# lijingzhu1/SKGHOI

Hardware: AMD Instinct MI355X
Metric: images/sec through interaction head (20x20 pairs) (higher is better)
Workload: dtype f32; 1 GPU; HICO-DET-shaped synthetic cached detections: 20 humans x 20 objects per image (G=800 grid rows, P=780 pairs, K=117 verbs), eval forward of InteractionHead from cached AdaMixer-R50 box features [40,256,7,7]/image; precision=fp32, batch_per_gpu=256, parallelism=dp1 (independent image shards, no data-path collective)

## Files before the change

include/skghoi.h:

```cpp
#ifndef SKGHOI_H
#define SKGHOI_H
#include <stdint.h>
#ifdef __cplusplus
extern "C" {
#endif

#define SKG_ABI_VERSION 19
#define SKG_E_ARG   (-1)
#define SKG_E_ALIGN (-2)
#define SKG_E_LIMIT (-3)
#define SKG_E_UNSUPPORTED (-4)
#define SKG_E_COMM  (-5)

#define SKG_MAX_DET_PER_IMAGE 1024
#define SKG_MAX_NODES         160
#define SKG_SPATIAL_LD        48
#define SKG_TRANSH_DIM        50
#define SKG_TRANSH_ENT        80

int         skg_abi_version(void);
const char* skg_build_info(void);

typedef struct {
    int32_t image;
// ... 117 lines not shown
int skg_gemm_dot_partials(const skg_gemm_desc* desc_host);

#define SKG_GEMM_GROUP_MAX 4
int skg_gemm_group_f32(const skg_gemm_desc* descs_host, int n, void* stream);
int skg_gemm_group_tile(const skg_gemm_desc* descs_host, int n);
int skg_gemm_b16_f32(const skg_gemm_desc* desc_host, const uint16_t* w16, void* stream);
int skg_gemm_group_b16_f32(const skg_gemm_desc* descs_host, const uint16_t* const* w16_host, int n, void* stream);
int skg_gemm_b16_a16_f32(const skg_gemm_desc* desc_host, const uint16_t* a16, const uint16_t* w16, void* stream);
void skg_gemm_b16_a16_launches(int64_t* out_host, int reset);
typedef struct {
    const uint16_t* w16;
    const uint16_t* a16;
    uint16_t*       c16; int64_t ldc16;
} skg_gemm_b16_io;
int  skg_gemm_b16_x(const skg_gemm_desc* desc_host, const skg_gemm_b16_io* io, void* stream);
int  skg_gemm_group_b16_x(const skg_gemm_desc* descs_host, const skg_gemm_b16_io* ios, int n, void* stream);
void skg_gemm_b16_x_counts(int64_t* out3, int reset);
#define SKG_GEMM_PATH_EXACT  0
#define SKG_GEMM_PATH_FP16X2 1
#define SKG_GEMM_PATH_BF16   2
#define SKG_GEMM_PATH_ROUTED 3
#define SKG_GEMM_PATHS       4
void skg_gemm_path_counts(int64_t* out_host, int reset);
typedef struct { int32_t small_mode, small_tiles, route_tiles, khalves_blocks; } skg_tuning;

int skg_concat_entity_f32(const float* enc, int64_t ld_enc, const int32_t* enc_row, const float* ent,
                          const int32_t* ent_img, const int32_t* ent_row, int rows, float* out, int64_t out_ld,
                          void* stream);
int skg_concat_entity_x(const float* enc, int64_t ld_enc, const int32_t* enc_row, const float* ent,
                        const int32_t* ent_img, const int32_t* ent_row, int rows, void* out, int64_t out_ld,
                        int out_dtype, void* stream);

typedef struct {
    const uint16_t* A; int64_t lda;
    const uint16_t* W; int64_t ldw;
    const float* bias;
    void* C; int64_t ldc;
    int32_t M, N, K;
    int32_t relu, out_bf16, split_k;
    float* split_ws;
} skg_gemm_bf16_desc;
int skg_gemm_bf16(const skg_gemm_bf16_desc* desc_host, void* stream);
int skg_transpose_bf16(const void* in, int64_t ld_in, int rows, int cols, void* out, int64_t ld_out, void* stream);

int skg_transpose_f32(const float* in, int64_t ld_in, int rows, int cols, float* out, int64_t ld_out, void* stream);

int skg_rows_mul_relu_f32(const float* P, const int32_t* p_idx, int64_t ldp, const float* Q, const int32_t* q_idx,
// ... 275 lines not shown
```

skghoi_amd/_capi.py:

```python
import ctypes as C
import os

_HERE = os.path.dirname(os.path.abspath(__file__))
LIB_PATH = os.environ.get("SKG_LIB") or os.path.join(_HERE, "csrc", "libskghoi_hip.so")

EPI_BIAS, EPI_BIAS_RELU, EPI_MUL_RELU, EPI_RELU_DOT, EPI_BIAS_RES_RELU = range(5)
DTYPE_F32, DTYPE_F16, DTYPE_BF16 = range(3)
DTYPE_BYTES = 3
CACHE_MAX_ARRAYS, CACHE_MAX_BATCH = 16, 256
MAX_DET_PER_IMAGE = 1024
MAX_NODES = 160
SPATIAL_LD = 48
TRANSH_DIM = 50
TRANSH_ENT = 80
ABI_VERSION = 19
GEMM_GROUP_MAX = 4
CHECKSUM_PARTIALS = 1024
LOSS_CHUNKS = 64

_vp = C.c_void_p
_i32 = C.c_int32
_i64 = C.c_int64
_f32 = C.c_float


class GemmDesc(C.Structure):
    _fields_ = [("A", _vp), ("lda", _i64), ("W", _vp), ("ldw", _i64), ("bias", _vp), ("C", _vp), ("ldc", _i64),
                ("M", _i32), ("N", _i32), ("K", _i32), ("epilogue", _i32), ("a_rows", _vp), ("out_rows", _vp),
                ("P", _vp), ("p_idx", _vp), ("ldp", _i64), ("Q", _vp), ("q_idx", _vp), ("ldq", _i64),
                ("mbias", _vp), ("C_raw", _vp), ("ldc_raw", _i64), ("dot_w", _vp), ("dot_partial", _vp),
                ("res", _vp), ("ldres", _i64), ("split_k", _i32), ("w_scale", _f32), ("split_ws", _vp), ("w_split", _vp),
                ("a_exp", _vp)]


class GemmB16Io(C.Structure):
    _fields_ = [("w16", _vp), ("a16", _vp), ("c16", _vp), ("ldc16", _i64)]


class GemmXDesc(C.Structure):
# ... 94 lines not shown
                                  _vp, C.c_int, C.c_int, C.c_int, _vp, C.c_int, _vp]),
    "skg_roi_align_nhwc_x": (C.c_int, [_vp, C.c_int, _vp, _vp, _vp, C.c_int, C.c_int, C.c_int, C.c_int, _f32, C.c_int,
                                       _vp, _vp, C.c_int, C.c_int, C.c_int, _vp, C.c_int, _vp]),
    "skg_roi_align_bwd_nhwc_f32": (C.c_int, [_vp, _vp, _vp, _vp, C.c_int, C.c_int, C.c_int, C.c_int, _f32, C.c_int, _vp,
                                             _vp, C.c_int, C.c_int, C.c_int, _vp, _vp]),
    "skg_roi_align_layout_counts": (None, [C.POINTER(_i64), C.c_int]),
    "skg_roi_align_bwd_det_x": (C.c_int, [_vp, C.c_int, _vp, _vp, _vp, C.c_int, C.c_int, C.c_int, C.c_int, _f32, C.c_int,
                                          _vp, _vp, C.c_int, C.c_int, C.c_int, C.c_int, _vp, _vp]),
    "skg_roi_align_bwd_det_nhwc_x": (C.c_int, [_vp, C.c_int, _vp, _vp, _vp, C.c_int, C.c_int, C.c_int, C.c_int, _f32,
                                               C.c_int, _vp, _vp, C.c_int, C.c_int, C.c_int, C.c_int, _vp, _vp]),
    "skg_roi_align_det_counts": (None, [C.POINTER(_i64), C.c_int]),
    "skg_global_avgpool_f32": (C.c_int, [_vp, C.c_int, C.c_int, C.c_int, _vp, _vp]),
    "skg_gemm_f32": (C.c_int, [C.POINTER(GemmDesc), _vp]),
    "skg_transh_draw_f32": (C.c_int, [_vp, _i64, C.c_int, C.c_int, C.c_int, C.c_int, _vp, _vp, _vp]),
    "skg_transh_draw_train_f32": (C.c_int, [_vp, _i64, C.c_int, C.c_int, C.c_int, _vp, _vp, _vp, _vp, _vp, _vp]),
    "skg_gemm_dot_partials": (C.c_int, [C.POINTER(GemmDesc)]),
    "skg_split_weights_bytes": (C.c_int64, [C.c_int, C.c_int]),
    "skg_split_weights_f16x2": (C.c_int, [_vp, C.c_int, C.c_int, _i64, _f32, _vp, _vp]),
    "skg_gemm_group_f32": (C.c_int, [C.POINTER(GemmDesc), C.c_int, _vp]),
    "skg_gemm_group_tile": (C.c_int, [C.POINTER(GemmDesc), C.c_int]),
    "skg_gemm_b16_f32": (C.c_int, [C.POINTER(GemmDesc), _vp, _vp]),
    "skg_gemm_group_b16_f32": (C.c_int, [C.POINTER(GemmDesc), C.POINTER(_vp), C.c_int, _vp]),
    "skg_gemm_path_counts": (None, [C.POINTER(_i64), C.c_int]),
    "skg_gemm_b16_a16_f32": (C.c_int, [C.POINTER(GemmDesc), _vp, _vp, _vp]),
    "skg_gemm_b16_a16_launches": (None, [C.POINTER(_i64), C.c_int]),
    "skg_gemm_b16_x": (C.c_int, [C.POINTER(GemmDesc), C.POINTER(GemmB16Io), _vp]),
    "skg_gemm_group_b16_x": (C.c_int, [C.POINTER(GemmDesc), C.POINTER(GemmB16Io), C.c_int, _vp]),
    "skg_gemm_b16_x_counts": (None, [C.POINTER(_i64), C.c_int]),
    "skg_row_exponents_f32": (C.c_int, [_vp, C.c_int64, _vp, C.c_int, C.c_int, _vp, _vp]),
    "skg_adamw_f32": (C.c_int, [_vp, C.c_int] + [C.c_double] * 7 + [_vp, C.c_int, _vp]),
    "skg_grad_sumsq_f32": (C.c_int, [_vp, C.c_int, _vp, _vp]),
    "skg_adamw_guarded_f32": (C.c_int, [_vp, C.c_int] + [C.c_double] * 7 + [_i64, C.c_double, C.c_int, _vp, C.c_int, _vp,
                                                                          C.c_int, _vp, _vp]),
    "skg_sizeof_step_status": (C.c_int, []),
    "skg_ctx_set_tuning": (C.c_int, [_vp, C.POINTER(Tuning)]),
    "skg_ctx_get_tuning": (C.c_int, [_vp, C.POINTER(Tuning)]),
    "skg_ctx_make_current": (_vp, [_vp]),
    "skg_gemmx_ws_floats": (C.c_int64, [C.POINTER(GemmXDesc)]),
    "skg_gemmx_f32": (C.c_int, [C.POINTER(GemmXDesc), C.c_int, _vp]),
    "skg_gemmx_bf16": (C.c_int, [C.POINTER(GemmXDesc), C.c_int, _vp]),
    "skg_gemmx_path_counts": (None, [C.POINTER(_i64), C.c_int]),
    "skg_gemm_bf16": (C.c_int, [C.POINTER(GemmBf16Desc), _vp]),
    "skg_transpose_bf16": (C.c_int, [_vp, _i64, C.c_int, C.c_int, _vp, _i64, _vp]),
    "skg_transpose_f32": (C.c_int, [_vp, _i64, C.c_int, C.c_int, _vp, _i64, _vp]),
    "skg_concat_entity_f32": (C.c_int, [_vp, _i64, _vp, _vp, _vp, _vp, C.c_int, _vp, _i64, _vp]),
    "skg_concat_entity_x": (C.c_int, [_vp, _i64, _vp, _vp, _vp, _vp, C.c_int, _vp, _i64, C.c_int, _vp]),
# ... 152 lines not shown
```

skghoi_amd/csrc/skg_common.h:

```cpp
#pragma once
#include <hip/hip_runtime.h>
#include <stdint.h>
#include "skghoi.h"

#define SKG_WAVE 64

typedef float f32x16 __attribute__((ext_vector_type(16)));
typedef float f32x4 __attribute__((ext_vector_type(4)));

static inline int skg_launch_status() {
    hipError_t e = hipGetLastError();
    return e == hipSuccess ? 0 : (int)e;
}

static inline bool skg_aligned16(const void* p) { return (((uintptr_t)p) & 15u) == 0; }
__device__ __forceinline__ bool skg_aligned16_dev(const void* p) { return (((uintptr_t)p) & 15u) == 0; }

__device__ __forceinline__ float skg_wave_sum(float v) {
#pragma unroll
    for (int off = 32; off > 0; off >>= 1) v += __shfl_xor(v, off, 64);
    return v;
}
__device__ __forceinline__ float skg_wave_max(float v) {
#pragma unroll
    for (int off = 32; off > 0; off >>= 1) v = fmaxf(v, __shfl_xor(v, off, 64));
    return v;
}

__device__ __forceinline__ float skg_block_sum256(float v, float* red) {
    v = skg_wave_sum(v);
    const int w = threadIdx.x >> 6;
    __syncthreads();
    if ((threadIdx.x & 63) == 0) red[w] = v;
    __syncthreads();
    return (red[0] + red[1]) + (red[2] + red[3]);
}

extern thread_local const skg_tuning* skg_tls_tuning;
static inline int skg_tune_small_mode() { const skg_tuning* t = skg_tls_tuning; return t && t->small_mode > 0 ? t->small_mode : 3; }
static inline int skg_tune_small_tiles() { const skg_tuning* t = skg_tls_tuning; return t && t->small_tiles > 0 ? t->small_tiles : 384; }
static inline int skg_tune_route_tiles() { const skg_tuning* t = skg_tls_tuning; return t && t->route_tiles > 0 ? t->route_tiles : 200; }
static inline int skg_tune_khalves_blocks() { const skg_tuning* t = skg_tls_tuning; return t && t->khalves_blocks > 0 ? t->khalves_blocks : 320; }

struct skg_twin_map { const float* base[2]; uint16_t* base16[2]; int64_t n[2]; };
extern thread_local skg_twin_map skg_tls_twin;
static inline uint16_t* skg_twin(const float* p) {
    const skg_twin_map& m = skg_tls_twin;
    for (int i = 0; i < 2; ++i)
        if (m.base16[i] && p >= m.base[i] && p < m.base[i] + m.n[i]) return m.base16[i] + (p - m.base[i]);
    return nullptr;
}
typedef __bf16 skg_bf2 __attribute__((ext_vector_type(2)));
typedef float skg_f2 __attribute__((ext_vector_type(2)));
__device__ __forceinline__ uint32_t skg_pack_bf16(float a, float b) {
    const skg_f2 v = {a, b};
    return __builtin_bit_cast(uint32_t, __builtin_convertvector(v, skg_bf2));
}
__device__ __forceinline__ void skg_store_twin4(uint16_t* p, const float4 v) {
    *reinterpret_cast<uint2*>(p) = make_uint2(skg_pack_bf16(v.x, v.y), skg_pack_bf16(v.z, v.w));
}

struct skg_gemmx_fused {
    int kind;
    const float* P; const int32_t* p_idx; int64_t ldp;
    const float* Q; const int32_t* q_idx; int64_t ldq;
    const float* mbias;
    float* C_raw; int64_t ldc_raw;
    const int32_t* out_rows;
    const float* res; int64_t ldres;
};
int skg_gemmx_can_fuse(const skg_gemmx_desc* d, const skg_gemmx_fused* f);
int skg_gemmx_f32_fused(const skg_gemmx_desc* descs_host, const skg_gemmx_fused* fused_host, int n, void* stream);

#define SKG_MULTI_MAX 4
struct skg_rows_mul_args {
    const float* P; const int32_t* p_idx; int64_t ldp; const float* Q; const int32_t* q_idx; int64_t ldq; const float* mbias;
    const float* F; const int32_t* f_idx; int64_t ldf; int rows, cols; float* out; int64_t ldo;
    uint16_t* out16;
};
int skg_rows_mul_relu_multi(const skg_rows_mul_args* calls, int n, void* stream);
struct skg_mul_bwd_args {
    float* g; int64_t ldg; const float* F; const int32_t* f_idx; int64_t ldf; const float* P; const int32_t* p_idx; int64_t ldp;
    const float* Q; const int32_t* q_idx; int64_t ldq; const float* mbias; int rows; float* dF; int64_t lddf; int accumulate;
    uint16_t* dF16;
};
int skg_mul_bwd_multi(const skg_mul_bwd_args* calls, int n, void* stream);
struct skg_segment_sum_args {
    const float* src; int64_t ld; int mode; float* outH; float* outN; int accumulate;
    uint16_t* outH16; uint16_t* outN16;
};
int skg_segment_sum_multi(const skg_segment_sum_args* calls, int n, const skg_image_meta* meta, const int32_t* hum_img,
                          const int32_t* node_img, int sum_h, int sum_n, void* stream);
struct skg_add_layernorm_args {
    const float* a; int64_t lda; const float* b; int64_t ldb; const float* gamma; const float* beta; int rows;
// ... 17 lines not shown
```

skghoi_amd/csrc/skg_gemm.hip:

```cpp
#include "skg_common.h"
#include <string.h>
#include <atomic>
#include <type_traits>

__device__ __forceinline__ float skg_exp2i(int e) { return __uint_as_float((uint32_t)(127 + e) << 23); }

typedef _Float16 f16x8 __attribute__((ext_vector_type(8)));
typedef _Float16 h16x2 __attribute__((ext_vector_type(2)));
typedef uint32_t u32x4 __attribute__((ext_vector_type(4)));
typedef short s16x8 __attribute__((ext_vector_type(8)));
typedef __bf16 bf16x2_t __attribute__((ext_vector_type(2)));
typedef float f32x2_t __attribute__((ext_vector_type(2)));

__device__ __forceinline__ uint32_t skg_pack_bf16x2(float a, float b) {
    const f32x2_t v = {a, b};
    return __builtin_bit_cast(uint32_t, __builtin_convertvector(v, bf16x2_t));
}
__device__ __forceinline__ void skg_store_bf16x4(uint16_t* p, float a, float b, float c, float e) {
    *reinterpret_cast<uint2*>(p) = make_uint2(skg_pack_bf16x2(a, b), skg_pack_bf16x2(c, e));
}
__device__ __forceinline__ void skg_store_bf16(uint16_t* p, float a) { *p = (uint16_t)(skg_pack_bf16x2(a, 0.f) & 0xffffu); }

#define BM 128
#define BN 128
// ... 1248 lines not shown
    if (d.split_k > 1 && (!d.split_ws || (d.epilogue != SKG_EPI_BIAS && d.epilogue != SKG_EPI_BIAS_RELU &&
                                          d.epilogue != SKG_EPI_BIAS_RES_RELU) || d.split_k > 64))
        return SKG_E_ARG;
    if (d.M < 0 || d.N <= 0 || d.K <= 0 || !d.A || !d.W) return SKG_E_ARG;
    if ((d.K & 3) || (d.lda & 3) || (d.ldw & 3)) return SKG_E_ALIGN;
    if (!skg_aligned16(d.A) || !skg_aligned16(d.W)) return SKG_E_ALIGN;
    if (d.lda < d.K && !d.a_rows && d.M > 1) return SKG_E_ARG;
    switch (d.epilogue) {
        case SKG_EPI_BIAS: case SKG_EPI_BIAS_RELU:
            if (!d.C) return SKG_E_ARG; break;
        case SKG_EPI_MUL_RELU:
            if (!d.C || (!d.P && !d.Q)) return SKG_E_ARG; break;
        case SKG_EPI_RELU_DOT:
            if (!d.dot_w || !d.dot_partial) return SKG_E_ARG; break;
        case SKG_EPI_BIAS_RES_RELU:
            if (!d.C || !d.res) return SKG_E_ARG; break;
        default: return SKG_E_ARG;
    }
    return 0;
}

#define g_route_tiles skg_tune_route_tiles()

static bool skg_route_desc(const skg_gemm_desc& d, skg_gemmx_desc& x, skg_gemmx_fused& f) {
    if (d.w_split || d.a_rows || d.a_exp || d.epilogue == SKG_EPI_RELU_DOT) return false;
    memset(&x, 0, sizeof(x)); memset(&f, 0, sizeof(f));
    x.A = d.A; x.a_sm = d.lda; x.a_sk = 1;
    x.B = d.W; x.b_sn = d.ldw; x.b_sk = 1;
    x.C = d.C; x.ldc = d.ldc; x.M = d.M; x.N = d.N; x.K = d.K;
    x.bias = d.bias; x.relu = d.epilogue == SKG_EPI_BIAS_RELU ? 1 : 0;
    x.split_k = d.split_k > 1 ? d.split_k : 0; x.split_ws = d.split_ws;
    f.out_rows = d.out_rows;
    if (d.epilogue == SKG_EPI_MUL_RELU) {
        f.kind = SKG_EPI_MUL_RELU;
        f.P = d.P; f.p_idx = d.p_idx; f.ldp = d.ldp; f.Q = d.Q; f.q_idx = d.q_idx; f.ldq = d.ldq; f.mbias = d.mbias;
        f.C_raw = d.C_raw; f.ldc_raw = d.ldc_raw;
    } else if (d.epilogue == SKG_EPI_BIAS_RES_RELU) {
        f.kind = SKG_EPI_BIAS_RES_RELU; f.res = d.res; f.ldres = d.ldres;
    }
    return skg_gemmx_can_fuse(&x, &f) != 0;
}

static bool skg_gemm_group_small(const skg_gemm_desc* descs, int n) {
    int64_t tiles128 = 0;
    for (int i = 0; i < n; ++i) {
        const skg_gemm_desc& d = descs[i];
        if (d.M == 0) continue;
        const bool glds = SKG_USE_GLDS && BK == 16 && (d.K % BK) == 0 && !d.a_rows &&
                          (int64_t)BM * d.lda * 4 < 0xffffffffLL && (int64_t)BN * d.ldw * 4 < 0xffffffffLL;
        if (!glds || (d.w_split && d.w_scale > 0.f)) return false;
        tiles128 += (int64_t)((d.M + 127) / 128) * ((d.N + 127) / 128);
    }
    return tiles128 < g_small_tiles;
}

static std::atomic<long long> g_gemm_path[SKG_GEMM_PATHS];
static inline void skg_gemm_count(int path) { g_gemm_path[path].fetch_add(1, std::memory_order_relaxed); }

extern "C" void skg_gemm_path_counts(int64_t* out_host, int reset) {
    for (int i = 0; i < SKG_GEMM_PATHS; ++i) {
        if (out_host) out_host[i] = g_gemm_path[i].load(std::memory_order_relaxed);
        if (reset) g_gemm_path[i].store(0, std::memory_order_relaxed);
    }
}

extern "C" int skg_gemm_group_tile(const skg_gemm_desc* descs_host, int n) {
    if (!descs_host || n < 1 || n > SKG_GEMM_GROUP_MAX) return SKG_E_ARG;
    return skg_gemm_group_small(descs_host, n) ? 1 : 2;
}

extern "C" int skg_gemm_group_f32(const skg_gemm_desc* descs_host, int n, void* stream) {
    if (!descs_host || n < 1 || n > SKG_GEMM_GROUP_MAX) return SKG_E_ARG;
    skg_gemm_group_args g, r;
    g.n = r.n = 0;
    int64_t blocks = 0, rblocks = 0;
    bool split = true;
    for (int i = 0; i < n; ++i) {
        const int rc = skg_gemm_validate(descs_host[i]);
        if (rc) return rc;
    }
    const bool small = skg_gemm_group_small(descs_host, n);
    if (n <= SKG_GEMMX_GROUP_MAX) {
        skg_gemmx_desc xs[SKG_GEMMX_GROUP_MAX];
        skg_gemmx_fused fs[SKG_GEMMX_GROUP_MAX];
        int64_t tiles128 = 0;
        bool ok = true;
        for (int i = 0; i < n && ok; ++i) {
            const skg_gemm_desc& d = descs_host[i];
            ok = skg_route_desc(d, xs[i], fs[i]);
            tiles128 += (int64_t)((d.M + 127) / 128) * ((d.N + 127) / 128) * (d.split_k > 1 ? d.split_k : 1);
        }
        if (ok && tiles128 >= g_route_tiles && tiles128 < 4 * g_small_tiles) {
            skg_gemm_count(SKG_GEMM_PATH_ROUTED);
            return skg_gemmx_f32_fused(xs, fs, n, stream);
        }
    }
    for (int i = 0; i < n; ++i) {
        const skg_gemm_desc& d = descs_host[i];
        if (d.split_k > 1 && !small) return SKG_E_ARG;
        if (d.M == 0) continue;
        split = split && d.w_split && (d.K % 16) == 0 && d.w_scale > 0.f;
        const int64_t nb = skg_gemm_blocks(d.M, d.N, d.K, small ? 1 : 2) * (d.split_k > 1 ? d.split_k : 1);
        if (blocks + nb > 0x7fffffffLL) return SKG_E_LIMIT;
        g.d[g.n] = d;
        g.start[g.n] = (int)blocks;
        blocks += nb;
        ++g.n;
        if (d.split_k > 1) {
            r.d[r.n] = d;
            r.start[r.n] = (int)rblocks;
            rblocks += ((int64_t)d.M * d.N + 255) / 256;
            ++r.n;
        }
    }
    if (g.n == 0) return 0;
// ... 5 lines not shown
    if (direct) hipLaunchKernelGGL(skg_gemm_group_direct_kernel, dim3((unsigned)blocks), dim3(256), 0, (hipStream_t)stream, g);
    else if (halves) hipLaunchKernelGGL(skg_gemm_group_khalves_kernel, dim3((unsigned)blocks), dim3(512), 0, (hipStream_t)stream, g);
    else if (small && g_small_mode >= 3) hipLaunchKernelGGL(skg_gemm_group_latency_kernel, dim3((unsigned)blocks), dim3(256), 0, (hipStream_t)stream, g);
    else if (small) hipLaunchKernelGGL(skg_gemm_group_small_kernel, dim3((unsigned)blocks), dim3(256), 0, (hipStream_t)stream, g);
    else if (split) hipLaunchKernelGGL(skg_gemm_group_split_kernel, dim3((unsigned)blocks), dim3(256), 0, (hipStream_t)stream, g);
    else hipLaunchKernelGGL(skg_gemm_group_kernel, dim3((unsigned)blocks), dim3(256), 0, (hipStream_t)stream, g);
    if (r.n) {
        for (int i = r.n; i <= SKG_GEMM_GROUP_MAX; ++i) r.start[i] = (int)rblocks;
        hipLaunchKernelGGL(skg_splitk_reduce_group_kernel, dim3((unsigned)rblocks), dim3(256), 0, (hipStream_t)stream, r);
    }
    return skg_launch_status();
}

extern "C" int skg_gemm_f32(const skg_gemm_desc* dh, void* stream) {
    if (!dh) return SKG_E_ARG;
    const skg_gemm_desc d = *dh;
    const int rc = skg_gemm_validate(d);
    if (rc) return rc;
    if (d.M == 0) return 0;
    const bool glds = SKG_USE_GLDS && BK == 16 && (d.K % BK) == 0 && !d.a_rows &&
                      (int64_t)BM * d.lda * 4 < 0xffffffffLL && (int64_t)BN * d.ldw * 4 < 0xffffffffLL;
    const bool split = d.w_split && (d.K % 16) == 0 && d.w_scale > 0.f;
    const int T = split ? 2 : skg_gemm_tile_scale(&d);
    if (!split && T == 1 && d.M > 64) {
        const int64_t tiles128 = (int64_t)((d.M + 127) / 128) * ((d.N + 127) / 128) * (d.split_k > 1 ? d.split_k : 1);
        skg_gemmx_desc x; skg_gemmx_fused f;
        if (tiles128 >= g_route_tiles && skg_route_desc(d, x, f)) {
            skg_gemm_count(SKG_GEMM_PATH_ROUTED);
            return skg_gemmx_f32_fused(&x, &f, 1, stream);
        }
    }
    const int64_t nblk = skg_gemm_blocks(d.M, d.N, d.K, T) * (d.split_k > 1 ? d.split_k : 1);
    if (nblk > 0x7fffffffLL) return SKG_E_LIMIT;
    dim3 grid((unsigned)nblk), block(256);
    hipStream_t s = (hipStream_t)stream;
    skg_gemm_count(split ? SKG_GEMM_PATH_FP16X2 : SKG_GEMM_PATH_EXACT);
#define SKG_LAUNCH(E)                                                                              \
    if (split) hipLaunchKernelGGL((skg_gemm_kernel<E, 2, 2>), grid, block, 0, s, d);               \
    else if (glds && T == 1 && g_small_mode == 4 && (d.K % 64) == 0) hipLaunchKernelGGL((skg_gemm_kernel<E, 4, 1>), grid, block, 0, s, d); \
    else if (glds && T == 1 && (g_small_mode == 5 || (g_small_mode == 6 && nblk <= g_khalves_blocks))) hipLaunchKernelGGL((skg_gemm_kernel<E, 5, 1>), grid, dim3(512), 0, s, d); \
    else if (glds && T == 1 && g_small_mode >= 3) hipLaunchKernelGGL((skg_gemm_kernel<E, 3, 1>), grid, block, 0, s, d); \
    else if (glds && T == 1) hipLaunchKernelGGL((skg_gemm_kernel<E, 1, 1>), grid, block, 0, s, d); \
    else if (glds) hipLaunchKernelGGL((skg_gemm_kernel<E, 1, 2>), grid, block, 0, s, d);           \
    else hipLaunchKernelGGL((skg_gemm_kernel<E, 0, 2>), grid, block, 0, s, d);
    switch (d.epilogue) {
        case SKG_EPI_BIAS:          SKG_LAUNCH(SKG_EPI_BIAS) break;
        case SKG_EPI_BIAS_RELU:     SKG_LAUNCH(SKG_EPI_BIAS_RELU) break;
        case SKG_EPI_MUL_RELU:      SKG_LAUNCH(SKG_EPI_MUL_RELU) break;
        case SKG_EPI_RELU_DOT:      SKG_LAUNCH(SKG_EPI_RELU_DOT) break;
        case SKG_EPI_BIAS_RES_RELU: SKG_LAUNCH(SKG_EPI_BIAS_RES_RELU) break;
// ... 306 lines not shown
```

skghoi_amd/csrc/skg_gemm_x.hip:

```cpp
#include "skg_common.h"
#include <stdlib.h>
#include <string.h>
#include <type_traits>
#include <atomic>

#define XBM 128
#define XBN 128
#define XBK 16
#define XLD 130
#define XTILE (XBK * XLD)
#ifndef SKG_XXCD
#define SKG_XXCD 1
#endif

struct skg_gemmx_group {
    skg_gemmx_desc d[SKG_GEMMX_GROUP_MAX];
    int start[SKG_GEMMX_GROUP_MAX + 1];
    skg_gemmx_fused f[SKG_GEMMX_GROUP_MAX];
    int vec[SKG_GEMMX_GROUP_MAX];
    int n;
};

__device__ __forceinline__ int64_t xoff(int idx, int shift, int64_t bstride, int64_t estride) {
    if (shift <= 0) return (int64_t)idx * estride;
// ... 169 lines not shown
}

template <bool WT = false>
__device__ __forceinline__ void xep_rows(const skg_gemmx_desc& d, const skg_gemmx_fused& f, const float* stage, int lane,
                                         int row0, int col0, float* ws) {
    const int c4 = 4 * (lane & 15), rr = lane >> 4, col = col0 + c4;
    if (col >= d.N) return;
    const bool hb = !ws && d.bias;
    float4 bv = xzero4(), mb = xzero4();
    if (hb) bv = xld4(d.bias + col);
    if (f.kind == SKG_EPI_MUL_RELU && f.mbias) mb = xld4(f.mbias + col);
    const int64_t coff = xoff(col, d.c_nshift, d.c_nstride, 1);
#pragma unroll
    for (int i = 0; i < 8; ++i) {
        const int row = row0 + 4 * i + rr;
        if (row >= d.M) continue;
        const float4 v = *reinterpret_cast<const float4*>(stage + (4 * i + rr) * XEP_LD + c4);
        if (WT) { xst_sc1(xrsrc(ws), ((uint32_t)row * (uint32_t)d.N + (uint32_t)col) * 4u, v); continue; }
        if (ws) { *reinterpret_cast<float4*>(ws + (int64_t)row * d.N + col) = v; continue; }
        xep_apply(d, f, v, row, col, coff, hb, bv, mb);
    }
}

template <bool OWN, int R>
__device__ __forceinline__ void xep_reduce(const skg_gemmx_desc& d, const skg_gemmx_fused& f, const float* stage, int lane,
                                           int row0, int col0, const XRed& red) {
    static_assert(R == 4 || R == 8, "rows per lane and pass");
    const int c4 = 4 * (lane & 15), rr = lane >> 4, col = col0 + c4;
    if (col >= d.N) return;
    const bool hb = d.bias != nullptr;
    float4 bv = xzero4(), mb = xzero4();
    if (hb) bv = xld4(d.bias + col);
    if (f.kind == SKG_EPI_MUL_RELU && f.mbias) mb = xld4(f.mbias + col);
    const int64_t coff = xoff(col, d.c_nshift, d.c_nstride, 1);
#pragma unroll 1
    for (int h = 0; h < 8 / R; ++h) {
        uint32_t ro[R];
        float4 sum[R];
#pragma unroll
        for (int i = 0; i < R; ++i) {
            ro[i] = ((uint32_t)min(row0 + 4 * (R * h + i) + rr, d.M - 1) * (uint32_t)d.N + (uint32_t)col) * 4u;
            sum[i] = xzero4();
        }
        auto add_slices = [&](int s0, int s1) {
            int s = s0;
            for (; s + 1 < s1; s += 2) {
// ... 247 lines not shown
    const bool split = S > 1;
    const int64_t MN = (int64_t)d.M * d.N;
    float* ws = split ? d.split_ws + (int64_t)slice * MN : nullptr;
    const bool inl = split && d.split_ctr != nullptr;
    if (c.do_rowsum && tid < XBM && m0 + tid < d.M) {
        if (split) xstore_rowsum_part(d.split_ws + (int64_t)S * MN + (int64_t)slice * d.M + m0 + tid, rsum, inl);
        else d.a_rowsum[m0 + tid] = d.accumulate ? d.a_rowsum[m0 + tid] + rsum : rsum;
    }
    if (vecbits & 8) {
        float* stage = smem + wave * XEP_WAVE;
#pragma unroll
        for (int ps = 0; ps < 2; ++ps) {
#pragma unroll
            for (int g2 = 0; g2 < 2; ++g2)
#pragma unroll
                for (int t = 0; t < 4; ++t)
#pragma unroll
                    for (int mb = 0; mb < 2; ++mb) {
                        const int e = 4 * (2 * ps + g2) + t;
                        *reinterpret_cast<float2*>(stage + (2 * (8 * g2 + 4 * lk + t) + mb) * XEP_LD + 2 * li) =
                            make_float2(acc[mb][0][e], acc[mb][1][e]);
                    }
            if (inl) xep_rows<true>(d, g.f[gi], stage, lane, m0 + wm * 64 + 32 * ps, n0 + wn * 64, ws);
            else xep_rows(d, g.f[gi], stage, lane, m0 + wm * 64 + 32 * ps, n0 + wn * 64, ws);
        }
        if (!inl || !xsplit_last(d.split_ctr + tm * nbn + tn, S, reinterpret_cast<uint32_t*>(smem + XEP_FLOATS))) return;
        if (c.do_rowsum && tid < XBM && m0 + tid < d.M) xreduce_rowsum_sc1(d, MN, m0 + tid);
        const XRed red = {d.split_ws, MN, S, -1};
#pragma unroll 1
        for (int ps = 0; ps < 2; ++ps)
            xep_reduce<false, 4>(d, g.f[gi], stage, lane, m0 + wm * 64 + 32 * ps, n0 + wn * 64, red);
        return;
    }
    const bool vecC = (vecbits >> 2) & 1;
    const int col = n0 + wn * 64 + 2 * li;
#pragma unroll
    for (int gq = 0; gq < 4; ++gq)
#pragma unroll
        for (int t = 0; t < 4; ++t)
#pragma unroll
            for (int mb = 0; mb < 2; ++mb) {
                const int row = m0 + wm * 64 + 2 * (8 * gq + 4 * lk + t) + mb;
                if (row >= d.M || col >= d.N) continue;
                float v0 = acc[mb][0][4 * gq + t], v1 = acc[mb][1][4 * gq + t];
                if (split) {
                    float* p = ws + (int64_t)row * d.N + col;
// ... 868 lines not shown
    if (quads) {
        const int64_t i = 4 * w;
        float4 v = xzero4();
        for (int s = 0; s < d.split_k; ++s) {
            const float4 q = xld4(d.split_ws + (int64_t)s * MN + i);
            v.x += q.x; v.y += q.y; v.z += q.z; v.w += q.w;
        }
        const int row = (int)(i / d.N), col = (int)(i % d.N);
        if (d.bias) { const float4 bv = xld4(d.bias + col); v.x += bv.x; v.y += bv.y; v.z += bv.z; v.w += bv.w; }
        if (d.relu) { v.x = fmaxf(v.x, 0.f); v.y = fmaxf(v.y, 0.f); v.z = fmaxf(v.z, 0.f); v.w = fmaxf(v.w, 0.f); }
        float* p = d.C + xoff(col, d.c_nshift, d.c_nstride, 1) + (int64_t)row * d.ldc;
        if (d.accumulate) { const float4 o = xld4(p); v.x += o.x; v.y += o.y; v.z += o.z; v.w += o.w; }
        if (d.mask) {
            const float4 m = xld4(d.mask + (int64_t)row * d.ldmask + col);
            v.x = m.x > 0.f ? v.x : 0.f; v.y = m.y > 0.f ? v.y : 0.f; v.z = m.z > 0.f ? v.z : 0.f; v.w = m.w > 0.f ? v.w : 0.f;
        }
        *reinterpret_cast<float4*>(p) = v;
        if (d.C16) *reinterpret_cast<uint2*>(d.C16 + (p - d.C)) = make_uint2(ypack(v.x, v.y), ypack(v.z, v.w));
        return;
    }
    xreduce_elem(d, MN, (int)(w / d.N), (int)(w % d.N));
}

static int skg_gemmx_validate(const skg_gemmx_desc& d) {
    if (d.M < 0 || d.N < 0 || d.K < 0) return SKG_E_ARG;
    if (d.M == 0 || d.N == 0) return 0;
    if (!d.C || d.ldc < 1) return SKG_E_ARG;
    if (d.K > 0 && (!d.A || !d.B)) return SKG_E_ARG;
    if (d.a_sm != 1 && d.a_sk != 1) return SKG_E_ARG;
    if (d.b_sn != 1 && d.b_sk != 1) return SKG_E_ARG;
    if (d.b_kshift < 0 || d.b_kshift > 30 || d.b_nshift < 0 || d.b_nshift > 30 || d.c_nshift < 0 || d.c_nshift > 30)
        return SKG_E_ARG;
    if ((d.b_kshift == 1) || (d.b_nshift == 1)) return SKG_E_ARG;
    if (d.mask && d.ldmask < d.N) return SKG_E_ARG;
    if (d.split_k > 1 && (!d.split_ws || d.split_k > 256)) return SKG_E_ARG;
    if ((((uintptr_t)d.C16) & 1u) || (((uintptr_t)d.A16) & 1u) || (((uintptr_t)d.B16) & 1u)) return SKG_E_ALIGN;
    if (((uintptr_t)d.split_ctr) & 3u) return SKG_E_ALIGN;
    if (d.a16_ld < 0 || d.b16_ld < 0 || (d.b16_ld && (d.b_kshift || d.b_nshift))) return SKG_E_ARG;
    if (d.a16_ld && d.a16_ld < (d.a_sk == 1 ? d.K : d.M)) return SKG_E_ARG;
    if (d.b16_ld && d.b16_ld < (d.b_sk == 1 ? d.K : d.N)) return SKG_E_ARG;
    return 0;
}

static bool xmul4(int64_t v) { return (v & 3) == 0; }
static bool xmul8(int64_t v) { return (v & 7) == 0; }

static int64_t xspan(int64_t idx, int shift, int64_t bstride, int64_t estride) {
    if (idx <= 0) return 0;
    if (shift <= 0) return idx * estride;
    return (idx >> shift) * bstride + (idx & ((1LL << shift) - 1)) * estride;
}
static bool xfits32(int64_t elems) { return elems >= 0 && elems < (1LL << 29); }

extern "C" int64_t skg_gemmx_ws_floats(const skg_gemmx_desc* d) {
    if (!d) return SKG_E_ARG;
    return d->split_k > 1 ? (int64_t)d->split_k * ((int64_t)d->M * d->N + d->M) : 0;
}

static bool xfused_ptrs_ok(const skg_gemmx_fused& f) {
    return skg_aligned16(f.P) && skg_aligned16(f.Q) && skg_aligned16(f.mbias) && skg_aligned16(f.C_raw) &&
           skg_aligned16(f.res) && xmul4(f.ldp) && xmul4(f.ldq) && xmul4(f.ldc_raw) && xmul4(f.ldres);
}

static std::atomic<long long> g_path_launches[3];
extern "C" void skg_gemmx_path_counts(int64_t* out3_host, int reset) {
    for (int i = 0; i < 3; ++i) {
        if (out3_host) out3_host[i] = g_path_launches[i].load(std::memory_order_relaxed);
        if (reset) g_path_launches[i].store(0, std::memory_order_relaxed);
    }
}

static bool g_t16_enabled = getenv("SKG_GEMMX_T16") == nullptr || atoi(getenv("SKG_GEMMX_T16")) != 0;

static int skg_gemmx_launch(const skg_gemmx_desc* descs_host, int n, void* stream, bool bf16,
                            const skg_gemmx_fused* fused_host = nullptr) {
    if (!descs_host || n < 1 || n > SKG_GEMMX_GROUP_MAX) return SKG_E_ARG;
    skg_gemmx_group g, r;
    memset(g.f, 0, sizeof(g.f)); memset(r.f, 0, sizeof(r.f));
    g.n = r.n = 0;
    int64_t blocks = 0, rblocks = 0;
    for (int i = 0; i < n; ++i) {
        const skg_gemmx_desc& d = descs_host[i];
        const int rc = skg_gemmx_validate(d);
        if (rc) return rc;
        if (d.M == 0 || d.N == 0) continue;
        const int S = d.split_k > 1 ? d.split_k : 1;
        const int64_t nb = (int64_t)((d.M + XBM - 1) / XBM) * ((d.N + XBN - 1) / XBN) * S;
        if (blocks + nb > 0x7fffffffLL) return SKG_E_LIMIT;
        int vec = 0;
        if (skg_aligned16(d.A) && (d.a_sk == 1 ? xmul4(d.a_sm) : xmul4(d.a_sk)) &&
            xfits32((int64_t)(d.M - 1) * d.a_sm + (int64_t)(d.K - 1) * d.a_sk + 4))
            vec |= 1;
        if (skg_aligned16(d.B) && (d.b_sk == 1 ? xmul4(d.b_sn) : xmul4(d.b_sk)) &&
            (d.b_kshift == 0 || (xmul4(d.b_kstride) && d.b_kshift >= 5)) && (d.b_nshift == 0 || xmul4(d.b_nstride)) &&
            xfits32(xspan(d.N - 1, d.b_nshift, d.b_nstride, d.b_sn) + xspan(d.K - 1, d.b_kshift, d.b_kstride, d.b_sk) + 4))
            vec |= 2;
        if ((((uintptr_t)d.C) & 7u) == 0 && (d.ldc & 1) == 0 && (d.c_nshift == 0 || (d.c_nstride & 1) == 0)) vec |= 4;
        if ((d.N & 3) == 0 && skg_aligned16(d.C) && xmul4(d.ldc) &&
            (d.c_nshift == 0 || (d.c_nshift >= 2 && xmul4(d.c_nstride))) && skg_aligned16(d.bias) &&
            skg_aligned16(d.mask) && (!d.mask || xmul4(d.ldmask)) && (S == 1 || skg_aligned16(d.split_ws)) &&
            (((uintptr_t)d.C16) & 7u) == 0)
            vec |= 8;
        const int64_t lda16 = d.a16_ld ? d.a16_ld : (d.a_sk == 1 ? d.a_sm : d.a_sk);
        const int64_t ldb16 = d.b16_ld ? d.b16_ld : (d.b_sk == 1 ? d.b_sn : d.b_sk);
        if (bf16 && d.A16 && ((vec & 1) || d.a16_ld) && skg_aligned16(d.A16) && xmul8(lda16) &&
            xfits32((int64_t)(d.a_sk == 1 ? d.M : d.K) * lda16 + 8))
            vec |= 16;
        if (bf16 && d.B16 && ((vec & 2) || d.b16_ld) && skg_aligned16(d.B16) && xmul8(ldb16) &&
            (d.b_kshift == 0 || xmul8(d.b_kstride)) && (d.b_nshift == 0 || (d.b_nshift >= 3 && xmul8(d.b_nstride))) &&
// ... 33 lines not shown
        for (int i = 0; i < g.n; ++i) {
            if (g.d[i].a16_ld) g.vec[i] &= ~16;
            if (g.d[i].b16_ld) g.vec[i] &= ~32;
        }
    g_path_launches[t16 ? 2 : (bf16 ? 1 : 0)].fetch_add(1, std::memory_order_relaxed);
    if (t16) hipLaunchKernelGGL(skg_gemmx_t16_kernel, dim3((unsigned)blocks), dim3(256), 0, (hipStream_t)stream, g);
    else if (bf16) hipLaunchKernelGGL(skg_gemmx_bf16_kernel, dim3((unsigned)blocks), dim3(256), 0, (hipStream_t)stream, g);
    else hipLaunchKernelGGL(skg_gemmx_kernel, dim3((unsigned)blocks), dim3(256), 0, (hipStream_t)stream, g);
    if (r.n) {
        for (int i = r.n; i <= SKG_GEMMX_GROUP_MAX; ++i) r.start[i] = (int)rblocks;
        hipLaunchKernelGGL(skg_gemmx_reduce_kernel, dim3((unsigned)rblocks), dim3(256), 0, (hipStream_t)stream, r);
    }
    return skg_launch_status();
}

extern "C" int skg_gemmx_f32(const skg_gemmx_desc* descs_host, int n, void* stream) {
    return skg_gemmx_launch(descs_host, n, stream, false);
}

int skg_gemmx_f32_fused(const skg_gemmx_desc* descs_host, const skg_gemmx_fused* fused_host, int n, void* stream) {
    return skg_gemmx_launch(descs_host, n, stream, false, fused_host);
}

int skg_gemmx_can_fuse(const skg_gemmx_desc* dp, const skg_gemmx_fused* f) {
    const skg_gemmx_desc& d = *dp;
    if (skg_gemmx_validate(d)) return 0;
    const bool staged = (d.N & 3) == 0 && skg_aligned16(d.C) && xmul4(d.ldc) && d.c_nshift == 0 && skg_aligned16(d.bias);
    if (!f || !(f->kind || f->out_rows)) return 1;
    return staged && (d.split_k <= 1 || d.split_ctr) && !d.accumulate && !d.mask && xfused_ptrs_ok(*f);
}

extern "C" int skg_gemmx_bf16(const skg_gemmx_desc* descs_host, int n, void* stream) {
    return skg_gemmx_launch(descs_host, n, stream, true);
}
```

Measured before the change: 8377 images/s.

## Route large GEMMs to gemmx kernel and add fused ReLU-dot epilogue

```diff
diff --git a/include/skghoi.h b/include/skghoi.h
--- a/include/skghoi.h
+++ b/include/skghoi.h
@@ -163,7 +163,16 @@
 #define SKG_GEMM_PATH_ROUTED 3
 #define SKG_GEMM_PATHS       4
 void skg_gemm_path_counts(int64_t* out_host, int reset);
+#define SKG_ROUTE_MID_ONLY  (-1)
+#define SKG_ROUTE_LARGE_ALL (-2)
 typedef struct { int32_t small_mode, small_tiles, route_tiles, khalves_blocks; } skg_tuning;
+#define SKG_GEMM_ROUTE_MODE0  0
+#define SKG_GEMM_ROUTE_MODE1  1
+#define SKG_GEMM_ROUTE_SMALL  2
+#define SKG_GEMM_ROUTE_FP16X2 3
+#define SKG_GEMM_ROUTE_MID    4
+#define SKG_GEMM_ROUTE_LARGE  5
+int skg_gemm_route_query(const skg_gemm_desc* descs_host, int n);
 
 int skg_concat_entity_f32(const float* enc, int64_t ld_enc, const int32_t* enc_row, const float* ent,
                           const int32_t* ent_img, const int32_t* ent_row, int rows, float* out, int64_t out_ld,
diff --git a/skghoi_amd/_capi.py b/skghoi_amd/_capi.py
--- a/skghoi_amd/_capi.py
+++ b/skghoi_amd/_capi.py
@@ -15,6 +15,8 @@
 TRANSH_ENT = 80
 ABI_VERSION = 19
 GEMM_GROUP_MAX = 4
+ROUTE_MID_ONLY, ROUTE_LARGE_ALL = -1, -2
+ROUTE_MODE0, ROUTE_MODE1, ROUTE_SMALL, ROUTE_FP16X2, ROUTE_MID, ROUTE_LARGE = range(6)
 CHECKSUM_PARTIALS = 1024
 LOSS_CHUNKS = 64
 
@@ -155,6 +157,7 @@
     "skg_gemm_b16_f32": (C.c_int, [C.POINTER(GemmDesc), _vp, _vp]),
     "skg_gemm_group_b16_f32": (C.c_int, [C.POINTER(GemmDesc), C.POINTER(_vp), C.c_int, _vp]),
     "skg_gemm_path_counts": (None, [C.POINTER(_i64), C.c_int]),
+    "skg_gemm_route_query": (C.c_int, [C.POINTER(GemmDesc), C.c_int]),
     "skg_gemm_b16_a16_f32": (C.c_int, [C.POINTER(GemmDesc), _vp, _vp, _vp]),
     "skg_gemm_b16_a16_launches": (None, [C.POINTER(_i64), C.c_int]),
     "skg_gemm_b16_x": (C.c_int, [C.POINTER(GemmDesc), C.POINTER(GemmB16Io), _vp]),
diff --git a/skghoi_amd/csrc/skg_common.h b/skghoi_amd/csrc/skg_common.h
--- a/skghoi_amd/csrc/skg_common.h
+++ b/skghoi_amd/csrc/skg_common.h
@@ -40,6 +40,7 @@
 static inline int skg_tune_small_mode() { const skg_tuning* t = skg_tls_tuning; return t && t->small_mode > 0 ? t->small_mode : 3; }
 static inline int skg_tune_small_tiles() { const skg_tuning* t = skg_tls_tuning; return t && t->small_tiles > 0 ? t->small_tiles : 384; }
 static inline int skg_tune_route_tiles() { const skg_tuning* t = skg_tls_tuning; return t && t->route_tiles > 0 ? t->route_tiles : 200; }
+static inline int skg_tune_route_select() { const skg_tuning* t = skg_tls_tuning; return t && t->route_tiles < 0 ? t->route_tiles : 0; }
 static inline int skg_tune_khalves_blocks() { const skg_tuning* t = skg_tls_tuning; return t && t->khalves_blocks > 0 ? t->khalves_blocks : 320; }
 
 struct skg_twin_map { const float* base[2]; uint16_t* base16[2]; int64_t n[2]; };
@@ -68,8 +69,9 @@
     float* C_raw; int64_t ldc_raw;
     const int32_t* out_rows;
     const float* res; int64_t ldres;
+    const float* dot_w; float* dot_partial;
 };
-int skg_gemmx_can_fuse(const skg_gemmx_desc* d, const skg_gemmx_fused* f);
+int skg_gemmx_can_fuse(const skg_gemmx_desc* d, const skg_gemmx_fused* f, int need_staged = 0);
 int skg_gemmx_f32_fused(const skg_gemmx_desc* descs_host, const skg_gemmx_fused* fused_host, int n, void* stream);
 
 #define SKG_MULTI_MAX 4
diff --git a/skghoi_amd/csrc/skg_gemm.hip b/skghoi_amd/csrc/skg_gemm.hip
--- a/skghoi_amd/csrc/skg_gemm.hip
+++ b/skghoi_amd/csrc/skg_gemm.hip
@@ -1294,8 +1294,33 @@
 
 #define g_route_tiles skg_tune_route_tiles()
 
-static bool skg_route_desc(const skg_gemm_desc& d, skg_gemmx_desc& x, skg_gemmx_fused& f) {
-    if (d.w_split || d.a_rows || d.a_exp || d.epilogue == SKG_EPI_RELU_DOT) return false;
+static bool skg_route_fits32(int rows, int64_t ld, int K) {
+    return (int64_t)(rows - 1) * ld + K + 3 < (1LL << 29);
+}
+
+enum { SKG_LARGE_MUL = 0, SKG_LARGE_MUL_RAW, SKG_LARGE_MUL_SCATTER, SKG_LARGE_WIDE_C, SKG_LARGE_DOT, SKG_LARGE_SHORT_K,
+       SKG_LARGE_LONG_K, SKG_LARGE_PLAIN, SKG_LARGE_UNMEASURED, SKG_LARGE_GROUP, SKG_LARGE_CLASSES };
+static int skg_large_class(const skg_gemm_desc& d) {
+    if (d.K < 512) return SKG_LARGE_SHORT_K;
+    if (d.K >= 4096) return SKG_LARGE_LONG_K;
+    if (d.epilogue == SKG_EPI_RELU_DOT) return SKG_LARGE_DOT;
+    if (d.epilogue == SKG_EPI_MUL_RELU) return d.out_rows ? SKG_LARGE_MUL_SCATTER : d.C_raw ? SKG_LARGE_MUL_RAW : SKG_LARGE_MUL;
+    if ((d.epilogue == SKG_EPI_BIAS || d.epilogue == SKG_EPI_BIAS_RELU) && !d.out_rows)
+        return d.ldc > d.N ? SKG_LARGE_WIDE_C : SKG_LARGE_PLAIN;
+    return SKG_LARGE_UNMEASURED;
+}
+static const bool g_large_default[SKG_LARGE_CLASSES] = {
+     true,  true,  false,  true,  true,  false,
+     true,  true,  false,  true };
+static bool skg_large_wanted(int cls) {
+    const int sel = skg_tune_route_select();
+    if (sel == SKG_ROUTE_MID_ONLY || g_route_tiles >= (1 << 30)) return false;
+    return sel == SKG_ROUTE_LARGE_ALL || g_large_default[cls];
+}
+
+static bool skg_route_desc(const skg_gemm_desc& d, skg_gemmx_desc& x, skg_gemmx_fused& f, bool large = false) {
+    if (d.w_split || d.a_rows || d.a_exp || (d.epilogue == SKG_EPI_RELU_DOT && !large)) return false;
+    if (large && (!skg_route_fits32(d.M, d.lda, d.K) || !skg_route_fits32(d.N, d.ldw, d.K))) return false;
     memset(&x, 0, sizeof(x)); memset(&f, 0, sizeof(f));
     x.A = d.A; x.a_sm = d.lda; x.a_sk = 1;
     x.B = d.W; x.b_sn = d.ldw; x.b_sk = 1;
@@ -1309,8 +1334,12 @@
         f.C_raw = d.C_raw; f.ldc_raw = d.ldc_raw;
     } else if (d.epilogue == SKG_EPI_BIAS_RES_RELU) {
         f.kind = SKG_EPI_BIAS_RES_RELU; f.res = d.res; f.ldres = d.ldres;
-    }
-    return skg_gemmx_can_fuse(&x, &f) != 0;
+    } else if (d.epilogue == SKG_EPI_RELU_DOT) {
+        f.kind = SKG_EPI_RELU_DOT; f.dot_w = d.dot_w; f.dot_partial = d.dot_partial;
+        f.out_rows = nullptr;
+        if (!d.C) x.ldc = d.N;
+    }
+    return skg_gemmx_can_fuse(&x, &f, large ? 1 : 0) != 0;
 }
 
 static bool skg_gemm_group_small(const skg_gemm_desc* descs, int n) {
@@ -1326,6 +1355,55 @@
     return tiles128 < g_small_tiles;
 }
 
+static int skg_route_group(const skg_gemm_desc* descs, int n, skg_gemmx_desc* xs, skg_gemmx_fused* fs) {
+    if (n > SKG_GEMMX_GROUP_MAX) return 0;
+    int64_t tiles128 = 0;
+    for (int i = 0; i < n; ++i)
+        tiles128 += (int64_t)((descs[i].M + 127) / 128) * ((descs[i].N + 127) / 128) * (descs[i].split_k > 1 ? descs[i].split_k : 1);
+    const bool large = tiles128 >= 4 * (int64_t)g_small_tiles;
+    if (large ? !skg_large_wanted(SKG_LARGE_GROUP) : tiles128 < g_route_tiles) return 0;
+    for (int i = 0; i < n; ++i) {
+        const skg_gemm_desc& d = descs[i];
+        if (large && d.M > 0 && (d.K % 16) != 0) return 0;
+        if (!skg_route_desc(d, xs[i], fs[i], large)) return 0;
+    }
+    return large ? 2 : 1;
+}
+
+static int skg_route_single(const skg_gemm_desc& d, skg_gemmx_desc& x, skg_gemmx_fused& f) {
+    const bool glds = SKG_USE_GLDS && BK == 16 && (d.K % BK) == 0 && !d.a_rows &&
+                      (int64_t)BM * d.lda * 4 < 0xffffffffLL && (int64_t)BN * d.ldw * 4 < 0xffffffffLL;
+    if (d.w_split && (d.K % 16) == 0 && d.w_scale > 0.f) return SKG_GEMM_ROUTE_FP16X2;
+    const int T = skg_gemm_tile_scale(&d);
+    const int64_t tiles128 = (int64_t)((d.M + 127) / 128) * ((d.N + 127) / 128) * (d.split_k > 1 ? d.split_k : 1);
+    if (T == 1 && d.M > 64 && tiles128 >= g_route_tiles && skg_route_desc(d, x, f)) return SKG_GEMM_ROUTE_MID;
+    if (T == 2 && glds && tiles128 >= g_small_tiles && skg_large_wanted(skg_large_class(d)) && skg_route_desc(d, x, f, true))
+        return SKG_GEMM_ROUTE_LARGE;
+    return !glds ? SKG_GEMM_ROUTE_MODE0 : T == 1 ? SKG_GEMM_ROUTE_SMALL : SKG_GEMM_ROUTE_MODE1;
+}
+
+extern "C" int skg_gemm_route_query(const skg_gemm_desc* descs_host, int n) {
+    if (!descs_host || n < 1 || n > SKG_GEMM_GROUP_MAX) return SKG_E_ARG;
+    for (int i = 0; i < n; ++i) {
+        const int rc = skg_gemm_validate(descs_host[i]);
+        if (rc) return rc;
+    }
+    skg_gemmx_desc xs[SKG_GEMMX_GROUP_MAX];
+    skg_gemmx_fused fs[SKG_GEMMX_GROUP_MAX];
+    if (n == 1) return skg_route_single(descs_host[0], xs[0], fs[0]);
+    const int r = skg_route_group(descs_host, n, xs, fs);
+    if (r) return r == 2 ? SKG_GEMM_ROUTE_LARGE : SKG_GEMM_ROUTE_MID;
+    if (skg_gemm_group_small(descs_host, n)) return SKG_GEMM_ROUTE_SMALL;
+    bool split = true, glds = true;
+    for (int i = 0; i < n; ++i) {
+        const skg_gemm_desc& d = descs_host[i];
+        if (d.M == 0) continue;
+        split = split && d.w_split && (d.K % 16) == 0 && d.w_scale > 0.f;
+        glds = glds && SKG_USE_GLDS && BK == 16 && (d.K % BK) == 0 && !d.a_rows;
+    }
+    return split ? SKG_GEMM_ROUTE_FP16X2 : glds ? SKG_GEMM_ROUTE_MODE1 : SKG_GEMM_ROUTE_MODE0;
+}
+
 static std::atomic<long long> g_gemm_path[SKG_GEMM_PATHS];
 static inline void skg_gemm_count(int path) { g_gemm_path[path].fetch_add(1, std::memory_order_relaxed); }
 
@@ -1352,17 +1430,10 @@
         if (rc) return rc;
     }
     const bool small = skg_gemm_group_small(descs_host, n);
-    if (n <= SKG_GEMMX_GROUP_MAX) {
+    {
         skg_gemmx_desc xs[SKG_GEMMX_GROUP_MAX];
         skg_gemmx_fused fs[SKG_GEMMX_GROUP_MAX];
-        int64_t tiles128 = 0;
-        bool ok = true;
-        for (int i = 0; i < n && ok; ++i) {
-            const skg_gemm_desc& d = descs_host[i];
-            ok = skg_route_desc(d, xs[i], fs[i]);
-            tiles128 += (int64_t)((d.M + 127) / 128) * ((d.N + 127) / 128) * (d.split_k > 1 ? d.split_k : 1);
-        }
-        if (ok && tiles128 >= g_route_tiles && tiles128 < 4 * g_small_tiles) {
+        if (skg_route_group(descs_host, n, xs, fs)) {
             skg_gemm_count(SKG_GEMM_PATH_ROUTED);
             return skg_gemmx_f32_fused(xs, fs, n, stream);
         }
@@ -1414,10 +1485,10 @@
                       (int64_t)BM * d.lda * 4 < 0xffffffffLL && (int64_t)BN * d.ldw * 4 < 0xffffffffLL;
     const bool split = d.w_split && (d.K % 16) == 0 && d.w_scale > 0.f;
     const int T = split ? 2 : skg_gemm_tile_scale(&d);
-    if (!split && T == 1 && d.M > 64) {
-        const int64_t tiles128 = (int64_t)((d.M + 127) / 128) * ((d.N + 127) / 128) * (d.split_k > 1 ? d.split_k : 1);
+    if (!split) {
         skg_gemmx_desc x; skg_gemmx_fused f;
-        if (tiles128 >= g_route_tiles && skg_route_desc(d, x, f)) {
+        const int route = skg_route_single(d, x, f);
+        if (route == SKG_GEMM_ROUTE_MID || route == SKG_GEMM_ROUTE_LARGE) {
             skg_gemm_count(SKG_GEMM_PATH_ROUTED);
             return skg_gemmx_f32_fused(&x, &f, 1, stream);
         }
diff --git a/skghoi_amd/csrc/skg_gemm_x.hip b/skghoi_amd/csrc/skg_gemm_x.hip
--- a/skghoi_amd/csrc/skg_gemm_x.hip
+++ b/skghoi_amd/csrc/skg_gemm_x.hip
@@ -215,6 +215,29 @@
     }
 }
 
+__device__ __forceinline__ void xep_rows_dot(const skg_gemmx_desc& d, const skg_gemmx_fused& f, const float* stage, int lane,
+                                             int row0, int col0, int slab) {
+    const int c4 = 4 * (lane & 15), rr = lane >> 4, col = col0 + c4;
+    const bool cin = col < d.N;
+    float4 bv = xzero4(), dw = xzero4();
+    if (cin) {
+        if (d.bias) bv = xld4(d.bias + col);
+        dw = xld4(f.dot_w + col);
+    }
+#pragma unroll
+    for (int i = 0; i < 8; ++i) {
+        const int row = row0 + 4 * i + rr;
+        const bool rin = row < d.M;
+        float4 v = *reinterpret_cast<const float4*>(stage + (4 * i + rr) * XEP_LD + c4);
+        v = make_float4(fmaxf(v.x + bv.x, 0.f), fmaxf(v.y + bv.y, 0.f), fmaxf(v.z + bv.z, 0.f), fmaxf(v.w + bv.w, 0.f));
+        float s = cin ? (v.x * dw.x + v.y * dw.y) + (v.z * dw.z + v.w * dw.w) : 0.f;
+        if (d.C && cin && rin) *reinterpret_cast<float4*>(d.C + (int64_t)row * d.ldc + col) = v;
+#pragma unroll
+        for (int off = 8; off > 0; off >>= 1) s += __shfl_xor(s, off, 64);
+        if ((lane & 15) == 0 && rin) f.dot_partial[(int64_t)slab * d.M + row] = s;
+    }
+}
+
 template <bool OWN, int R>
 __device__ __forceinline__ void xep_reduce(const skg_gemmx_desc& d, const skg_gemmx_fused& f, const float* stage, int lane,
                                            int row0, int col0, const XRed& red) {
@@ -508,6 +531,7 @@
                             make_float2(acc[mb][0][e], acc[mb][1][e]);
                     }
             if (inl) xep_rows<true>(d, g.f[gi], stage, lane, m0 + wm * 64 + 32 * ps, n0 + wn * 64, ws);
+            else if (g.f[gi].kind == SKG_EPI_RELU_DOT) xep_rows_dot(d, g.f[gi], stage, lane, m0 + wm * 64 + 32 * ps, n0 + wn * 64, tn * 2 + wn);
             else xep_rows(d, g.f[gi], stage, lane, m0 + wm * 64 + 32 * ps, n0 + wn * 64, ws);
         }
         if (!inl || !xsplit_last(d.split_ctr + tm * nbn + tn, S, reinterpret_cast<uint32_t*>(smem + XEP_FLOATS))) return;
@@ -1422,10 +1446,10 @@
     xreduce_elem(d, MN, (int)(w / d.N), (int)(w % d.N));
 }
 
-static int skg_gemmx_validate(const skg_gemmx_desc& d) {
+static int skg_gemmx_validate(const skg_gemmx_desc& d, bool need_c = true) {
     if (d.M < 0 || d.N < 0 || d.K < 0) return SKG_E_ARG;
     if (d.M == 0 || d.N == 0) return 0;
-    if (!d.C || d.ldc < 1) return SKG_E_ARG;
+    if ((need_c && !d.C) || d.ldc < 1) return SKG_E_ARG;
     if (d.K > 0 && (!d.A || !d.B)) return SKG_E_ARG;
     if (d.a_sm != 1 && d.a_sk != 1) return SKG_E_ARG;
     if (d.b_sn != 1 && d.b_sk != 1) return SKG_E_ARG;
@@ -1459,7 +1483,8 @@
 
 static bool xfused_ptrs_ok(const skg_gemmx_fused& f) {
     return skg_aligned16(f.P) && skg_aligned16(f.Q) && skg_aligned16(f.mbias) && skg_aligned16(f.C_raw) &&
-           skg_aligned16(f.res) && xmul4(f.ldp) && xmul4(f.ldq) && xmul4(f.ldc_raw) && xmul4(f.ldres);
+           skg_aligned16(f.res) && xmul4(f.ldp) && xmul4(f.ldq) && xmul4(f.ldc_raw) && xmul4(f.ldres) &&
+           skg_aligned16(f.dot_w) && (f.kind != SKG_EPI_RELU_DOT || (f.dot_w && f.dot_partial));
 }
 
 static std::atomic<long long> g_path_launches[3];
@@ -1481,10 +1506,12 @@
     int64_t blocks = 0, rblocks = 0;
     for (int i = 0; i < n; ++i) {
         const skg_gemmx_desc& d = descs_host[i];
-        const int rc = skg_gemmx_validate(d);
+        const bool dot = fused_host && fused_host[i].kind == SKG_EPI_RELU_DOT;
+        const int rc = skg_gemmx_validate(d, !dot);
         if (rc) return rc;
         if (d.M == 0 || d.N == 0) continue;
         const int S = d.split_k > 1 ? d.split_k : 1;
+        if (dot && S > 1) return SKG_E_ARG;
         const int64_t nb = (int64_t)((d.M + XBM - 1) / XBM) * ((d.N + XBN - 1) / XBN) * S;
         if (blocks + nb > 0x7fffffffLL) return SKG_E_LIMIT;
         int vec = 0;
@@ -1564,11 +1591,14 @@
     return skg_gemmx_launch(descs_host, n, stream, false, fused_host);
 }
 
-int skg_gemmx_can_fuse(const skg_gemmx_desc* dp, const skg_gemmx_fused* f) {
+int skg_gemmx_can_fuse(const skg_gemmx_desc* dp, const skg_gemmx_fused* f, int need_staged) {
     const skg_gemmx_desc& d = *dp;
-    if (skg_gemmx_validate(d)) return 0;
-    const bool staged = (d.N & 3) == 0 && skg_aligned16(d.C) && xmul4(d.ldc) && d.c_nshift == 0 && skg_aligned16(d.bias);
-    if (!f || !(f->kind || f->out_rows)) return 1;
+    const bool dot = f && f->kind == SKG_EPI_RELU_DOT;
+    if (skg_gemmx_validate(d, !dot)) return 0;
+    const bool staged = (d.N & 3) == 0 && skg_aligned16(d.C) && xmul4(d.ldc) && d.c_nshift == 0 && skg_aligned16(d.bias) &&
+                        (d.split_k <= 1 || skg_aligned16(d.split_ws));
+    if (!f || !(f->kind || f->out_rows)) return !need_staged || staged;
+    if (dot && d.split_k > 1) return 0;
     return staged && (d.split_k <= 1 || d.split_ctr) && !d.accumulate && !d.mask && xfused_ptrs_ok(*f);
 }
 
```

Result: no change. 8395 images/s, median of 2 (+0.2%).
